# brian-kelley/CUDA-QR

Hardware: AMD Instinct MI355X
Metric: fp64 GFLOP/s (% of roofline) + ||A-QR||_F/||A||_F, m x n QR at 1/2/4/8 GPUs (higher is better)
Workload: dtype f64; 1 GPU; C3: 16384x16384 square fp64 QR on 1 MI355X, nb=256; m=16384, n=16384, m_per_gpu=16384, nb=256, ib=32, input_buffers=31, input=uniform[0,1) counter-hash generator, seed 12+i, resident in HBM, collective=none

## Files before the change

### cuda-qr_amd/__init__.py

```python
import ctypes as C
import os

import numpy as np

HERE = os.path.dirname(os.path.abspath(__file__))
_which = os.environ.get("CUDA_QR_AMD_LIB", "")
LAB = _which == "lab" or _which.endswith(".so")
LAB_LIB_PATH = os.path.join(HERE, "libmi355xqr_lab.so")
LIB_PATH = (os.path.join(HERE, _which) if _which.endswith(".so") else LAB_LIB_PATH) if LAB else os.path.join(HERE, "libmi355xqr.so")
HEADER = os.path.join(os.path.dirname(HERE), "include", "mi355x_qr.h")

if not os.path.exists(LIB_PATH):
    raise ImportError(
        f"{LIB_PATH} is missing: build it with `make -C {HERE} all lab` (or python -c 'import __graft_entry__ as g; "
        "g.build()').  The HIP extension is mandatory; there is no CPU fallback.")

try:
    import torch
except Exception:
    pass

lib = C.CDLL(LIB_PATH)

QR_PROF_CLASSES = 4
# ... 243 lines not shown
_sig("qr_plan_get_profile", C.c_int, _vp, C.POINTER(Profile))
_sig("qr_plan_get_profile_records", C.c_int, _vp, C.c_int, C.POINTER(C.c_int), _dp, _dp)
_sig("qr_device_info", C.c_int, C.c_char_p, C.c_int, C.POINTER(C.c_int), C.POINTER(C.c_int), C.POINTER(C.c_size_t))
_sig("qr_probe_mfma_f64_tflops", C.c_int, _dp)
_sig("qr_probe_copy_gbps", C.c_int, _dp)
_sig("qrd_gemm_nn", C.c_int, _vp, C.c_int, C.c_int, C.c_int, C.c_double, _vp, C.c_int, _vp, C.c_int, C.c_double,
     _vp, C.c_int)
_sig("qrd_gemm_tn", C.c_int, _vp, C.c_int, C.c_int, C.c_int, C.c_double, _vp, C.c_int, _vp, C.c_int, C.c_double,
     _vp, C.c_int, _vp, C.c_size_t, _vp, C.c_int)
_sig("qrd_gemm_tn_update", C.c_int, _vp, C.c_int, C.c_int, C.c_int, C.c_double, _vp, C.c_int, _vp, C.c_int, C.c_double,
     _vp, C.c_int, _vp, C.c_size_t)
_sig("qrd_gemm_tn_update_wide", C.c_int, _vp, C.c_int, C.c_int, C.c_int, C.c_double, _vp, C.c_int, _vp, C.c_int, C.c_double,
     _vp, C.c_int, _vp, C.c_size_t)
if hasattr(lib, "qrd_gemm_tn_update_even"):
    _sig("qrd_gemm_tn_update_even", C.c_int, _vp, C.c_int, C.c_int, C.c_int, C.c_double, _vp, C.c_int, _vp, C.c_int, C.c_double,
         _vp, C.c_int, _vp, C.c_size_t, C.c_int)
    _sig("qrd_tn_even_launches", C.c_longlong)
    _sig("qrd_tn_even_last_grid", C.c_int)
if hasattr(lib, "qrd_gemm_nn_tri"):
    _sig("qrd_gemm_nn_tri", C.c_int, _vp, C.c_int, C.c_int, C.c_int, C.c_double, _vp, C.c_int, _vp, C.c_int, C.c_double,
         _vp, C.c_int)
    _sig("qrd_gemm_nn_tri_tile", C.c_int, _vp, C.c_int, C.c_int, C.c_int, C.c_int, _vp, C.c_int, _vp, C.c_int, _vp, C.c_int)
    _sig("qrd_vt_tri_launches", C.c_longlong)
_sig("qrd_gemm_tn_dual", C.c_int, _vp, C.c_int, C.c_int, C.c_int, _vp, C.c_int, _vp, C.c_int, _vp, C.c_int, _vp, C.c_int, _vp, C.c_int, _vp, C.c_int,
     _vp, C.c_size_t)
_sig("qrd_trsm_gt", C.c_int, _vp, C.c_int, C.c_int, _vp, C.c_int, _vp, C.c_int, _vp, C.c_int, _vp, C.c_int)
_sig("qrd_larft", C.c_int, _vp, C.c_int, C.c_int, _vp, C.c_int, _vp, _vp, C.c_int, _vp, C.c_int, _vp, C.c_int)
_sig("qrd_panel_ws_size", C.c_size_t, C.c_int)
_sig("qrd_panel_tsqr", C.c_int, _vp, _vp, C.c_int, C.c_int, C.c_int, _vp, _vp, C.c_int, _vp, C.c_int, _vp, C.c_int)
_sig("qrd_panel_cholqr", C.c_int, _vp, _vp, C.c_int, C.c_int, C.c_int, _vp, _vp, C.c_int, _vp, C.c_int, _vp, C.c_int, _vp, _vp, C.c_size_t, C.c_int)
_sig("qrd_leaf_update_gram", C.c_int, _vp, C.c_int, C.c_int, _vp, C.c_int, _vp, _vp, C.c_int, _vp, C.c_size_t, C.c_int, C.POINTER(C.c_int))
_sig("qrd_gemm_nt", C.c_int, _vp, C.c_int, C.c_int, C.c_int, C.c_int, _vp, C.c_int, _vp, C.c_int, _vp, C.c_int, C.c_int, _vp)
if hasattr(lib, "qrd_gemm_nt4_ok"):
    _sig("qrd_gemm_nt4_ok", C.c_int, C.c_int, C.c_int, C.c_int, _vp, C.c_int, _vp, C.c_int, _vp, C.c_int)
_sig("qrd_transpose", C.c_int, _vp, C.c_int, C.c_int, _vp, C.c_int, _vp, C.c_int)
_sig("qrd_copy_block", C.c_int, _vp, _vp, C.c_int, _vp, C.c_int, C.c_int, C.c_int)
_sig("qrd_init", C.c_int)
_sig("qrd_device_sync", C.c_int)


def strerror(rc):
    return lib.qr_strerror(rc).decode()


def check(rc, what=""):
    if rc != 0:
# ... 1484 lines not shown
```

### cuda-qr_amd/csrc/qr_host.c

```c
#define _POSIX_C_SOURCE 200809L
#include <pthread.h>
#include <sched.h>
#include <stdint.h>
#include <stdio.h>
#include <stdlib.h>
#include <string.h>
#include <time.h>

#include "../../include/mi355x_qr.h"
#include "qr_device.h"
#include "qr_plan_internal.h"

#define CHECK(x) do { int rc_ = (x); if (rc_) return rc_; } while (0)

#define QR_MAX_NB 512
#define QR_HALF 256
#define QR_DEFAULT_SPLIT "64"
#define QR_DEFAULT_SPLIT_BIG "32"

#define QR_MAX_DEVICES 64
static pthread_mutex_t g_lock = PTHREAD_MUTEX_INITIALIZER;
static int g_nb = 0, g_ib = 0;
static int g_nb_explicit = 0;
static unsigned char g_dev_inited[QR_MAX_DEVICES];

#define QR_FUSE_NN_MIN_ROWS 20000
#define QR_TFOLD_MAX 128
#define QR_EARLY_W1 4096
#define QR_TAIL_TC_MS 0.0

typedef struct qr_knobs {
    int fuse_nn;
    int split_t;
    int early_next;
    int plan_cache;
    int early_product;
    int fused_panel;
    int fused_min_rows;
    int tsqr_halves_rows;
    int cqr_min_rows;
    int tall_nt;
    int cqr_park;
    int cqr_min_rows_la;
    int cqr_retry;
    int trsm_next;
    int defer_t;
    int fused_gram;
} qr_knobs;
static qr_knobs g_knobs;
static pthread_once_t g_knobs_once = PTHREAD_ONCE_INIT;
// ... 249 lines not shown
        const char* b = lab_getenv("MI355XQR_BALANCE");
        p->bal_rp = 14.0; p->bal_ru = 44.0; p->bal_tc0 = 1.1; p->bal_tc1 = 0.6;
        if (p->npairs) {
            int cus = 256;
            qrd_device_info(NULL, 0, &cus, NULL, NULL);
            const int pc = qrd_stream_cus(p->s_pair[0][0]);
            p->bal_rp = 0.22 * pc; p->bal_ru = 0.244 * (cus - pc);
        }
        if (b) {
            p->bal_rp = 0.0;
            sscanf(b, "%lf,%lf,%lf,%lf", &p->bal_rp, &p->bal_ru, &p->bal_tc0, &p->bal_tc1);
        }
        {
            const char* tt = lab_getenv("MI355XQR_TAILTC");
            p->bal_tail_tc = tt ? atof(tt) : QR_TAIL_TC_MS;
        }
        p->bal_auto = (b == NULL) && p->npairs > 1;
        p->bal_tc0_base = p->bal_tc0; p->bal_tc1_base = p->bal_tc1;
    }
    for (int e = 0; e < 2 && !rc; ++e) rc = qrd_event_create_notiming(&p->ev_v[e]);
    for (int e = 0; e < 2 && !rc; ++e) {
        rc = qrd_event_create_notiming(&p->ev_panel[e]);
        if (!rc) rc = qrd_event_create_notiming(&p->ev_wide[e]);
        if (!rc) rc = qrd_event_create_notiming(&p->ev_tree[e]);
    }
    size_t cap = (size_t) 256 * nb * (size_t) n;
    if (cap > ((size_t) 16 << 20)) cap = (size_t) 16 << 20;
    if (cap < ((size_t) 1 << 16)) cap = (size_t) 1 << 16;
    p->slab_cap = cap;
    p->w_cap = (size_t) nb * n;
    for (int e = 0; e < 2 && !rc; ++e) {
        rc = qrd_malloc((void**) &p->Vw2[e], sizeof(double) * (size_t) p->ldv * nb);
        if (!rc) rc = qrd_malloc((void**) &p->VT2[e], sizeof(double) * (size_t) p->ldv * nb);
        if (!rc) rc = qrd_malloc((void**) &p->T2[e], sizeof(double) * (size_t) nb * nb);
        if (!rc) rc = qrd_memset(p->stream, p->T2[e], 0, sizeof(double) * (size_t) nb * nb);
        if (!rc) rc = qrd_memset(p->stream, p->Vw2[e], 0, sizeof(double) * (size_t) p->ldv * nb);
    }
    p->Vw = p->Vw2[0]; p->VT = p->VT2[0]; p->T = p->T2[0];
    if (!rc) rc = qrd_malloc((void**) &p->W, sizeof(double) * p->w_cap);
    if (!rc) rc = qrd_malloc((void**) &p->Wn, sizeof(double) * (size_t) nb * nb);
    if (!rc && p->npairs && p->bal_rp > 0.0) rc = qrd_malloc((void**) &p->We, sizeof(double) * p->w_cap);
    if (!rc && p->We) rc = qrd_malloc((void**) &p->Ye, sizeof(double) * p->w_cap);
    if (!rc) rc = qrd_malloc((void**) &p->Yn, sizeof(double) * (size_t) nb * nb);
    if (!rc && (size_t) n * 8 <= (size_t) m) rc = qrd_malloc((void**) &p->Ye2, sizeof(double) * p->w_cap);
    if (!rc) rc = qrd_malloc((void**) &p->slabs_u, sizeof(double) * p->slab_cap);
    if (!rc) rc = qrd_malloc((void**) &p->Tt, sizeof(double) * (size_t) nb * nb);
    if (!rc) rc = qrd_malloc((void**) &p->G, sizeof(double) * (size_t) nb * nb);
    if (!rc) rc = qrd_malloc((void**) &p->X, sizeof(double) * (size_t) nb * nb);
    if (!rc) rc = qrd_malloc((void**) &p->slabs, sizeof(double) * p->slab_cap);
    {
        const char* pa = getenv("MI355XQR_PANEL");
        p->panel_tsqr = (pa && strcmp(pa, "tsqr") == 0) ? 1 : 3;
    }
    if (!rc) rc = qrd_malloc((void**) &p->panel_ws, sizeof(double) * qrd_panel_ws_size(m));
    if (!rc && p->panel_tsqr == 3) rc = qrd_malloc((void**) &p->chol_ws, sizeof(double) * QRD_CHOLQR_WS);
    if (!rc && p->panel_tsqr == 3 && knobs()->early_product) {
        p->slab_ep_cap = (size_t) 32 * (size_t) (nb > 64 ? nb : 64) * 128;
        rc = qrd_malloc((void**) &p->slabs_ep, sizeof(double) * p->slab_ep_cap);
    }
    if (!rc && p->panel_tsqr == 3 && knobs()->fused_panel) {
        if (knobs()->cqr_min_rows > 0 && m >= plan_cqr_min_rows(p)) {
            rc = qrd_malloc((void**) &p->cq_ws, sizeof(double) * qrd_panel_cqr_ws_doubles());
            if (!rc) rc = qrd_malloc((void**) &p->cq_status, 4 * sizeof(int));
            if (!rc) rc = qrd_memset(p->stream, p->cq_status, 0, 4 * sizeof(int));
            if (!rc) rc = qrd_host_word_alloc(&p->cq_hword, &p->cq_hword_dev);
            {
                const char* gm = getenv("MI355XQR_GUARD");
                p->guard_latch = gm != NULL && strcmp(gm, "latch") == 0;
            }
        }
        if (!rc) rc = qrd_malloc((void**) &p->pf_ws, sizeof(double) * qrd_panel_fused_ws_doubles());
        if (!rc) rc = qrd_memset(p->stream, p->pf_ws, 0, sizeof(double) * qrd_panel_fused_ws_doubles());
        if (!rc) rc = qrd_malloc((void**) &p->pf_status, 4 * sizeof(int));
        if (!rc) rc = qrd_memset(p->stream, p->pf_status, 0, 4 * sizeof(int));
    }
    if (!rc && (p->m != p->m_user || p->n != p->n_user)) rc = qrd_malloc((void**) &p->padA, sizeof(double) * (size_t) p->m * p->n);
    if (!rc && p->n != p->n_user) rc = qrd_malloc((void**) &p->pad_tau, sizeof(double) * (size_t) p->n);
    if (rc) { qr_plan_destroy(p); return rc; }
    *out = p;
    return 0;
}

int qr_plan_destroy(qr_plan* p)
{
    if (!p) return 0;
    qr_plan_sync(p);
    qrd_graph_destroy(p->graph_exec);
    for (int e = 0; e < 2; ++e) {
        if (p->ev_panel[e]) qrd_event_destroy(p->ev_panel[e]);
        if (p->ev_v[e]) qrd_event_destroy(p->ev_v[e]);
        if (p->ev_wide[e]) qrd_event_destroy(p->ev_wide[e]);
        if (p->ev_tree[e]) qrd_event_destroy(p->ev_tree[e]);
        qrd_free(p->Vw2[e]); qrd_free(p->VT2[e]); qrd_free(p->T2[e]);
    }
    qrd_free(p->Wn); qrd_free(p->slabs_u); qrd_free(p->We); qrd_free(p->Ye); qrd_free(p->Yn); qrd_free(p->Ye2);
    for (int i = 0; i < p->npairs; ++i)
        for (int j = 0; j < 2; ++j)
            if (p->s_pair[i][j] && !(j == 1 && p->pair_shared_u[i])) qrd_stream_destroy(p->s_pair[i][j]);
    if (p->npairs == 0 && p->stream_u) qrd_stream_destroy(p->stream_u);
    for (int e = 0; e < 2; ++e) {
        if (p->ev_hop[e]) qrd_event_destroy(p->ev_hop[e]);
        if (p->ev_extra[e]) qrd_event_destroy(p->ev_extra[e]);
        if (p->ev_next[e]) qrd_event_destroy(p->ev_next[e]);
        if (p->ev_half[e]) qrd_event_destroy(p->ev_half[e]);
    }
    for (int i = 0; i < 2 * p->prof_cap; ++i)
        if (p->prof_ev && p->prof_ev[i]) qrd_event_destroy(p->prof_ev[i]);
    free(p->prof_ev); free(p->prof_cls); free(p->prof_flops); free(p->prof_bytes);
    qrd_free(p->W); qrd_free(p->Tt); qrd_free(p->G); qrd_free(p->X);
    qrd_free(p->slabs); qrd_free(p->panel_ws); qrd_free(p->chol_ws); qrd_free(p->slabs_ep);
    qrd_free(p->pf_ws); qrd_free(p->pf_status); qrd_free(p->cq_ws); qrd_free(p->cq_status); qrd_free(p->padA); qrd_free(p->pad_tau);
    qrd_host_word_free(p->cq_hword);
    qrd_free(p->pv_d); qrd_free(p->pv_i); qrd_free(p->pv_scatter);
    qrd_free(p->sv_d); qrd_free(p->sv_i); qrd_free(p->sv_t); free(p->sv_h);
    qrd_free(p->hd_status);
    if (p->s_main) qrd_stream_destroy(p->s_main);
    free(p);
    return 0;
}

static int plan_read_status(qr_plan* p)
{
    int rc = 0;
    if (p->pf_dirty && p->pf_status) {
        int st[4] = {0, 0, 0, 0};
        CHECK(qrd_d2h(p->s_main, st, p->pf_status, sizeof st));
        CHECK(qrd_stream_sync(p->s_main));
        p->pf_dirty = 0;
        if (st[0] || st[1]) {
            CHECK(qrd_memset(p->s_main, p->pf_status, 0, sizeof st));
            CHECK(qrd_stream_sync(p->s_main));
        }
// ... 334 lines not shown
        if (!need_t) continue;
        if (p->v_ready && nhalf == 1) CHECK(qrd_event_record(p->v_ready, p->stream));
        double* Vh = p->Vw + (size_t) c0 * ldv + c0;
        double* Thh = p->T + (size_t) c0 * ldt + c0;
        if (wh > ib && !cqr_done && p->defer_hint && fused_half && nhalf == 1 && !gram_done) {
            p->t_deferred = 1;
            continue;
        }
        if (wh > ib && !cqr_done) {
            double* Ghh = p->G + (size_t) c0 * nb + c0;
            if (!gram_done) CHECK(tn(p, wh, wh, mk - c0, Vh, ldv, Vh, ldv, Ghh, nb, NULL));
            if (!t_merged) CHECK(qrd_larft(p->stream, wh, ib, Ghh, nb, dtau + k + c0, Thh, ldt, NULL, 0, p->X, nb));
        }
        if (h > 0) {
            double* G12 = p->G + (size_t) c0 * nb;
            CHECK(tn(p, c0, wh, mk - c0, p->Vw + c0, ldv, Vh, ldv, G12, nb, NULL));
            CHECK(qrd_gemm_nn(p->stream, c0, wh, wh, 1.0, G12, nb, Thh, ldt, 0.0, p->X, c0));
            CHECK(qrd_gemm_nn(p->stream, c0, wh, c0, -1.0, p->T, ldt, p->X, c0, 0.0, p->T + (size_t) c0 * ldt, ldt));
        }
    }
    return 0;
}

static void use_set(qr_plan* p, int e) { p->Vw = p->Vw2[e]; p->VT = p->VT2[e]; p->T = p->T2[e]; }

static int apply_small_t(qr_plan* p, void* stream, const double* V, int ldv, const double* T, int ldt, int mk, int kw, double* A2,
                         int lda, int nc, double* Wbuf, double* Ybuf, double* slabs)
{
    void* const t_wait = p->t_wait;
    p->t_wait = NULL;
    const int fold_max = QR_TFOLD_MAX;
    if (kw <= fold_max && slabs != NULL) {
        if (t_wait) CHECK(qrd_stream_wait_event(stream, t_wait));
        CHECK(qrd_gemm_tn(stream, kw, nc, mk, 1.0, V, ldv, A2, lda, 0.0, Wbuf, kw, slabs, p->slab_cap, T, ldt));
    } else {
        CHECK(qrd_gemm_tn(stream, kw, nc, mk, 1.0, V, ldv, A2, lda, 0.0, Ybuf, kw, slabs, p->slab_cap, NULL, 0));
        if (t_wait) CHECK(qrd_stream_wait_event(stream, t_wait));
        CHECK(qrd_gemm_tn(stream, kw, nc, kw, 1.0, T, ldt, Ybuf, kw, 0.0, Wbuf, kw, NULL, 0, NULL, 0));
    }
    return apply_vw(p, stream, V, ldv, mk, kw, A2, lda, nc, Wbuf, Ybuf);
}

static int apply_vw(qr_plan* p, void* stream, const double* V, int ldv, int mk, int kw, double* A2, int lda, int nc, double* Wbuf, double* Ybuf)
{
    (void) p;
    if (knobs()->tall_nt && Ybuf && mk >= 16384 && kw >= 32 && kw % 16 == 0 && nc >= 128) {
        const int r = nc % 64, ni = nc - r;
// ... 108 lines not shown
    if (!p->npairs || p->bal_rp <= 0.0 || nwide <= 0) return 0;
    const double F = 4.0 * mk * (double) wout * 1e-9;
    const double tc = chain_ms(p, mk, wout);
    const double x = (F * nwide / p->bal_ru - tc) / (F * (1.0 / p->bal_rp + 1.0 / p->bal_ru));
    int xi = (int) x;
    xi -= xi % 128;
    if (xi < 128) return 0;
    return xi > nwide ? nwide : xi;
}

static int update_bound(const qr_plan* p, int mk, int wout, int nwide)
{
    if (!p->npairs || p->bal_ru <= 0.0 || nwide <= 0) return 0;
    const double F = 4.0 * mk * (double) wout * 1e-9;
    const double tc = chain_ms(p, mk, wout);
    return F * nwide / p->bal_ru > tc;
}

static int deferred_gram(qr_plan* p, void* stream, int e, int mk, int wout, double* slabs)
{
#ifdef QR_TRACE_DEFER
    fprintf(stderr, "deferred_t_merge: mk %d wout %d on %s\n", mk, wout, stream == p->stream_u ? "update stream" : "panel stream");
#endif
    return qrd_gemm_tn(stream, wout, wout, mk, 1.0, p->Vw2[e], p->ldv, p->Vw2[e], p->ldv, 0.0, p->G, p->nb, slabs, p->slab_cap, NULL, 0);
}
static int deferred_tree(qr_plan* p, void* stream, int e, int wout, const double* tau_k)
{
    return qrd_larft(stream, wout, p->ib, p->G, p->nb, tau_k, p->T2[e], p->ldt, NULL, 0, p->X, p->nb);
}
static int deferred_t_merge(qr_plan* p, void* stream, int e, int mk, int wout, const double* tau_k, double* slabs)
{
    CHECK(deferred_gram(p, stream, e, mk, wout, slabs));
    return deferred_tree(p, stream, e, wout, tau_k);
}

static int lookahead_update_no_t(qr_plan* p, void* stream, int e, double* dA, int lda, int k, int mk, int wout, int nc, double* slabs)
{
    double* A2 = dA + (size_t) (k + wout) * lda + k;
    if (wout % 32 || wout > 256 || nc % 16 || nc < 16 || p->ib != 32) return 1;
    CHECK(prof_begin_on(p, 4, stream));
    CHECK(qrd_gemm_tn(stream, wout, nc, mk, 1.0, p->Vw2[e], p->ldv, A2, lda, 0.0, p->Yn, wout, slabs, p->slab_cap, NULL, 0));
    CHECK(qrd_trsm_gt(stream, wout, nc, p->G, p->nb, p->T2[e], p->ldt, p->Yn, wout, p->Wn, wout));
    CHECK(apply_vw(p, stream, p->Vw2[e], p->ldv, mk, wout, A2, lda, nc, p->Wn, p->Yn));
    CHECK(prof_end(p, 4.0 * mk * (double) nc * wout, 24.0 * mk * (double) nc + 16.0 * mk * wout));
    return 0;
}

static int geqrf_issue(qr_plan* p, double* dA, int m, int n, int lda, double* dtau);

int qr_geqrf_dev(qr_plan* p, double* dA, int m, int n, int lda, double* dtau)
{
    if (!p || !dA || !dtau || n < 1 || m < n || m > p->m || n > p->n || lda < m) return QR_E_ARG;
    if (!p->padA && m == p->m_user && n == p->n_user && m >= 512 && !p->use_graph && !p->pad_failed && ((lda & 1) || ((uintptr_t) dA & 15)) &&
        (double) p->m * p->n * 8.0 <= 4294967296.0) {
        if (qrd_malloc((void**) &p->padA, sizeof(double) * (size_t) p->m * p->n)) { p->padA = NULL; p->pad_failed = 1; }
    }
    if (p->padA && m == p->m_user && n == p->n_user && !p->use_graph) {
        const int mp = p->m, np = p->n;
        CHECK(qrd_memset(p->stream, p->padA, 0, sizeof(double) * (size_t) mp * np));
        CHECK(qrd_copy_block(p->stream, dA, lda, p->padA, mp, m, n));
        if (np > n) CHECK(qrd_set_identity(p->stream, p->padA + (size_t) n * mp + m, mp, np - n, np - n, 0));
        CHECK(geqrf_issue(p, p->padA, mp, np, mp, np > n ? p->pad_tau : dtau));
        if (np > n) CHECK(qrd_d2d(p->stream, dtau, p->pad_tau, sizeof(double) * (size_t) n));
        return qrd_copy_block(p->stream, p->padA, mp, dA, lda, m, n);
    }
// ... 26 lines not shown
    void* ns = i < 0 ? p->s_main : p->s_pair[i][0];
    void* nu = i < 0 ? NULL : p->s_pair[i][1];
    CHECK(qrd_event_record(p->ev_hop[0], p->stream));
    CHECK(qrd_stream_wait_event(ns, p->ev_hop[0]));
    if (p->stream_u && p->stream_u != nu) {
        CHECK(qrd_event_record(p->ev_hop[1], p->stream_u));
        CHECK(qrd_stream_wait_event(nu ? nu : ns, p->ev_hop[1]));
    }
    p->stream = ns; p->stream_u = nu; p->pair_cur = i;
    if (i >= 0 && p->bal_auto) {
        int cus = 256;
        qrd_device_info(NULL, 0, &cus, NULL, NULL);
        const int pc = qrd_stream_cus(ns);
        const int uc = nu ? qrd_stream_cus(nu) : cus;
        p->bal_rp = 0.22 * (pc < cus ? pc : 32);
        p->bal_ru = 0.244 * uc;
        const double f = pc <= 32 ? 1.0 : (pc <= 64 ? 0.8 : 0.7);
        p->bal_tc0 = p->bal_tc0_base * f; p->bal_tc1 = p->bal_tc1_base * f;
    }
    return 0;
}

static int geqrf_issue_inner(qr_plan* p, double* dA, int m, int n, int lda, double* dtau);

static int geqrf_issue(qr_plan* p, double* dA, int m, int n, int lda, double* dtau)
{
    const int rc = geqrf_issue_inner(p, dA, m, n, lda, dtau);
    if (rc) {
        p->stream = p->s_main;
        p->stream_u = p->npairs ? NULL : p->stream_u;
        p->pair_cur = -1;
        use_set(p, 0);
    }
    return rc;
}

static int geqrf_issue_inner(qr_plan* p, double* dA, int m, int n, int lda, double* dtau)
{
    const int nb = p->nb;
    p->cq_parked = 0;
    p->park_hint = 0;
    p->defer_hint = 0;
    p->t_deferred = 0;
    if (!p->lookahead) {
        use_set(p, 0);
        for (int k = 0, wout = 0; k < n; k += wout) {
            wout = imin(nb, n - k);
            if (p->ib == 32 && wout > 32 && wout % 32 != 0) wout -= wout % 32;
            const int mk = m - k, nt = n - (k + wout);
            CHECK(prof_begin(p, 2));
            p->park_hint = nt == 0 || ((size_t) nt * 8 <= (size_t) mk && p->Ye2 != NULL);
            CHECK(factor_panel(p, dA, m, lda, k, wout, dtau, nt > 0, NULL));
            CHECK(prof_end(p, 2.0 * mk * (double) wout * wout, 16.0 * mk * wout));
            if (nt > 0) CHECK(update_cols(p, p->stream, 0, dA, lda, k, mk, wout, k + wout, nt, p->W, NULL, p->slabs, 1, 1));
            CHECK(cq_unpark(p));
        }
        return 0;
    }
    int wide_pending[2] = {0, 0}, extra_pending = 0;
    int v_recorded[2] = {0, 0};
    int t_deferred[2] = {0, 0};
    const int split_t = knobs()->split_t;
    const int early_env = knobs()->early_next, early_w1 = QR_EARLY_W1;
    int early_done = 0;
    {
        const int w0 = imin(nb, n);
        use_set(p, 0);
        CHECK(prof_begin(p, 2));
        p->v_ready = (split_t && p->npairs > 0 && w0 <= QR_HALF && n > w0) ? p->ev_v[0] : NULL;
        v_recorded[0] = p->v_ready != NULL;
        CHECK(factor_panel(p, dA, m, lda, 0, w0, dtau, n > w0, NULL));
        p->v_ready = NULL;
        CHECK(prof_end(p, 2.0 * m * (double) w0 * w0, 16.0 * m * w0));
        CHECK(qrd_event_record(p->ev_panel[0], p->stream));
    }
    CHECK(enter_phase(p, phase_of(p, n, n)));
    int s = 0;
    for (int k = 0; k < n; k += nb, ++s) {
        const int e = s & 1, wout = imin(nb, n - k), mk = m - k, nt = n - (k + wout);
        if (nt <= 0) break;
        const int wnext = imin(nb, nt), nwide = nt - wnext;
// ... 4 lines not shown
        CHECK(enter_phase(p, phase_now));
        int extra = p->We ? balance_cols(p, mk, wout, nwide) : 0;
        const int k1 = k + wout, mk1 = m - k1, nt1 = n - (k1 + wnext);
        const int wnext2 = nt1 > 0 ? imin(nb, nt1) : 0;
        const int early_next = early_env && p->npairs > 0 && p->stream_u != NULL && nhalf2 == 0 && wnext2 > 0 && wnext2 <= QR_HALF &&
                               nwide > wnext2 && update_bound(p, mk, wout, nwide) &&
                               update_bound(p, mk1, wnext, nt1 - wnext2) && phase_of(p, nt1, n) == phase_now;
        if (early_next && extra > nwide - wnext2) { extra = nwide - wnext2; extra -= extra % 128; }
        const int n_on_u = !n_early && p->stream_u != NULL && p->npairs > 0 &&
                           (p->next_on_update == 1 || (p->next_on_update == 2 && !update_bound(p, mk, wout, nwide)));
        if (t_deferred[e] && !n_on_u) {
            CHECK(deferred_t_merge(p, p->stream, e, mk, wout, dtau + k, p->slabs));
            CHECK(qrd_event_record(p->ev_panel[e], p->stream));
            t_deferred[e] = 0;
        }
        if (n_early) {
        } else if (n_on_u && t_deferred[e]) {
            CHECK(qrd_stream_wait_event(p->stream_u, v_recorded[e] ? p->ev_v[e] : p->ev_panel[e]));
            if (extra_pending) CHECK(qrd_stream_wait_event(p->stream_u, p->ev_extra[e ^ 1]));
            CHECK(prof_begin_on(p, 3, p->stream_u));
            CHECK(deferred_gram(p, p->stream_u, e, mk, wout, p->slabs_u));
            CHECK(prof_end(p, 2.0 * mk * (double) wout * wout, 8.0 * mk * wout));
            t_deferred[e] = 0;
            int need_tree_first = !knobs()->trsm_next;
            if (!need_tree_first) {
                const int rc = lookahead_update_no_t(p, p->stream_u, e, dA, lda, k, mk, wout, nfirst, p->slabs_u);
                if (rc < 0 || rc > 1) return rc;
                need_tree_first = rc == 1;
            }
            if (need_tree_first) {
                CHECK(deferred_tree(p, p->stream_u, e, wout, dtau + k));
                CHECK(update_cols(p, p->stream_u, e, dA, lda, k, mk, wout, k + wout, nfirst, p->Wn, p->Yn, p->slabs_u, 0, 0));
            }
            CHECK(qrd_event_record(p->ev_next[e], p->stream_u));
            CHECK(qrd_stream_wait_event(p->stream, p->ev_next[e]));
            if (!need_tree_first) {
                CHECK(deferred_tree(p, p->stream_u, e, wout, dtau + k));
                CHECK(qrd_event_record(p->ev_tree[e], p->stream_u));
                CHECK(qrd_stream_wait_event(p->stream, p->ev_tree[e]));
            }
            wide_pending[e ^ 1] = 0;
        } else if (n_on_u) {
            if (v_recorded[e]) {
                CHECK(qrd_stream_wait_event(p->stream_u, p->ev_v[e]));
                p->t_wait = p->ev_panel[e];
            } else
                CHECK(qrd_stream_wait_event(p->stream_u, p->ev_panel[e]));
            if (extra_pending) CHECK(qrd_stream_wait_event(p->stream_u, p->ev_extra[e ^ 1]));
            CHECK(update_cols(p, p->stream_u, e, dA, lda, k, mk, wout, k + wout, nfirst, p->Wn, p->Yn, p->slabs_u, 0, 0));
            p->t_wait = NULL;
            CHECK(qrd_event_record(p->ev_next[e], p->stream_u));
            CHECK(qrd_stream_wait_event(p->stream, p->ev_next[e]));
            wide_pending[e ^ 1] = 0;
        } else {
            if (s > 0 && wide_pending[e ^ 1]) {
                CHECK(qrd_stream_wait_event(p->stream, p->ev_wide[e ^ 1]));
                wide_pending[e ^ 1] = 0;
            }
            CHECK(update_cols(p, p->stream, e, dA, lda, k, mk, wout, k + wout, nfirst, p->Wn, p->Yn, p->slabs, 0, 0));
        }
        const int wide_cols = nhalf2 + nwide - extra;
        const int cw = k + wout + wnext;
        if (wide_cols > 0) {
// ... 39 lines not shown
        CHECK(prof_begin(p, 2));
        p->v_ready = (split_t && p->npairs > 0 && wnext <= QR_HALF && nt1 > 0) ? p->ev_v[e ^ 1] : NULL;
        v_recorded[e ^ 1] = p->v_ready != NULL;
        {
            const int nwide1 = nt1 - wnext2;
            const double w_ms = 4.0 * mk * (double) wout * (double) wide_cols * 1e-9 / (p->bal_ru > 0.0 ? p->bal_ru : 50.0);
            const int n_on_u1 = !early_next && p->stream_u != NULL && p->npairs > 0 &&
                                (p->next_on_update == 1 || (p->next_on_update == 2 && !update_bound(p, mk1, wnext, nwide1)));
            p->defer_hint = knobs()->defer_t && n_on_u1 && nt1 > 0 && wnext <= QR_HALF && w_ms < 0.75 * 0.45 * (double) wnext / 256.0 &&
                            phase_of(p, nt1, n) == phase_now;
        }
        CHECK(factor_panel(p, dA, m, lda, k1, wnext, dtau, nt1 > 0, nhalf2 > 0 ? p->ev_half[e] : NULL));
        p->defer_hint = 0;
        t_deferred[e ^ 1] = p->t_deferred;
        p->t_deferred = 0;
        p->v_ready = NULL;
        CHECK(prof_end(p, 2.0 * mk1 * (double) wnext * wnext, 16.0 * mk1 * wnext));
        CHECK(qrd_event_record(p->ev_panel[e ^ 1], p->stream));
        if (early_next) {
            CHECK(qrd_stream_wait_event(p->stream, p->ev_half[e]));
            CHECK(update_cols(p, p->stream, e ^ 1, dA, lda, k1, mk1, wnext, k1 + wnext, imin(QR_HALF, wnext2), p->Wn, p->Yn, p->slabs, 0, 0));
            early_done = 1;
        }
        if (extra > 0) {
            CHECK(update_cols(p, p->stream, e, dA, lda, k, mk, wout, early_next ? cw + nwide - extra : cw, extra, p->We, p->Ye,
                              p->slabs, 2, 0));
            CHECK(qrd_event_record(p->ev_extra[e], p->stream));
            extra_pending = 1;
        }
    }
    for (int e = 0; e < 2; ++e)
        if (wide_pending[e]) CHECK(qrd_stream_wait_event(p->stream, p->ev_wide[e]));
    use_set(p, 0);
    return enter_phase(p, -1);
}

int qr_applyq_dev(qr_plan* p, const double* dA, int m, int n, int lda, const double* dtau, double* dC, int ccols,
                  int ldc, int identity_start)
{
    if (!p || !dA || !dtau || !dC || n < 1 || m < n || m > p->m || n > p->n || ccols < 1 || ldc < m) return QR_E_ARG;
    const int nb = p->nb, ib = p->ib, ldv = p->ldv, ldt = p->ldt;
    CHECK(ensure_w(p, (size_t) nb * ccols));
    use_set(p, 0);
    if (identity_start) CHECK(qrd_set_identity(p->stream, dC, ldc, m, ccols, 0));
    const int npan = (n + nb - 1) / nb;
    for (int pi = npan - 1; pi >= 0; --pi) {
        const int k = pi * nb, wout = imin(nb, n - k), mk = m - k;
        const int c0 = identity_start ? k : 0, nc = ccols - c0;
        if (nc <= 0) continue;
        const double* Ak = dA + (size_t) k * lda + k;
        CHECK(qrd_extract_v(p->stream, Ak, lda, mk, wout, p->Vw, ldv));
        CHECK(tn(p, wout, wout, mk, p->Vw, ldv, p->Vw, ldv, p->G, nb, NULL));
        CHECK(qrd_larft(p->stream, wout, ib, p->G, nb, dtau + k, p->T, ldt, p->Tt, 1, p->X, nb));
        CHECK(qrd_gemm_nn(p->stream, mk, wout, wout, 1.0, p->Vw, ldv, p->Tt, ldt, 0.0, p->VT, ldv));
        double* Cs = dC + (size_t) c0 * ldc + k;
        CHECK(tn(p, wout, nc, mk, p->VT, ldv, Cs, ldc, p->W, wout, NULL));
        CHECK(qrd_gemm_nn(p->stream, mk, nc, wout, -1.0, p->Vw, ldv, p->W, wout, 1.0, Cs, ldc));
// ... 822 lines not shown
}

int qr_tsqr_is_pipelined(qr_tsqr_plan* t) { return t && t->pipe_ok && t->nranks > 1; }

int qr_tsqr_set_schedule(qr_tsqr_plan* t, int mode)
{
    if (!t || mode < 0 || mode > 2) return QR_E_ARG;
    if (t->nranks < 2) return 0;
    CHECK(qr_tsqr_sync(t));
    if (mode == 1 && !t->pipe_able) return QR_E_ARG;
    if (mode == 2) { t->pipe_ok = t->pipe_able && t->pipe_env_on; t->pipe_auto = t->pipe_env_auto; t->pipe_calls = 0; t->pipe_fell_back = 0; }
    else { t->pipe_ok = mode; t->pipe_auto = 0; }
    t->stats_valid = 0;
    return 0;
}

int qr_tsqr_factor_dev(qr_tsqr_plan* t, double* dA, int lda, double* dR)
{
    if (!t || !dA || !dR || lda < t->m_local) return QR_E_ARG;
    if (t->nranks > 1 && !t->comm) return QR_E_ARG;
    if (t->nranks > 1 && t->pipe_ok && t->pipe_auto && t->pipe_calls == QR_TSQR_DECIDE_CALL) CHECK(tsqr_decide(t, 0));
    if (t->nranks > 1 && t->pipe_ok) return tsqr_factor_pipelined(t, dA, lda, dR, 0);
    if (t->nranks == 1) {
        CHECK(qr_geqrf_dev(t->p, dA, t->m_local, t->n, lda, t->dtau));
        CHECK(qr_extract_r_dev(t->p, dA, t->m_local, t->n, lda, dR, t->n, t->n));
        t->local_done = 0;
        return 0;
    }
    CHECK(qr_tsqr_local_dev(t, dA, lda));
    CHECK(qrd_allgather_f64(t->comm, t->p->s_main, t->dRp, t->dRall, (size_t) t->n * t->n));
    return qr_tsqr_stacked_dev(t, dR);
}

int qr_tsqr_formq_dev(qr_tsqr_plan* t, const double* dA, int lda, double* dQ, int ldq)
{
    if (!t || !dA || !dQ || lda < t->m_local || ldq < t->m_local) return QR_E_ARG;
    const int n = t->n, rows = t->m_local, sm = t->sm;
    qr_plan* p = t->p;
    if (t->nranks == 1) return qr_applyq_dev(p, dA, rows, n, lda, t->dtau, dQ, n, ldq, 1);
    qr_plan* p2 = t->p2;
    if (t->ev_q && t->q_pending) { CHECK(qrd_stream_wait_event(p2->s_main, t->ev_q)); t->q_pending = 0; }
    CHECK(qr_applyq_dev(p2, t->dS, sm, n, sm, t->dtau2, t->dQt, n, sm, 1));
    CHECK(qrd_event_record(t->ev_stacked, p2->s_main));
    CHECK(qrd_stream_wait_event(p->s_main, t->ev_stacked));
    t->stacked_pending = 0;
    CHECK(qrd_zero_block(p->s_main, dQ, ldq, rows, n));
    CHECK(qrd_copy_block(p->s_main, t->dQt + (size_t) t->rank * n, sm, dQ, ldq, n, n));
    CHECK(qrd_event_record(t->ev_q, p->s_main));
// ... 106 lines not shown
```

### cuda-qr_amd/csrc/qr_kernels.hip

```cpp
#include <hip/hip_runtime.h>
#include <stdint.h>
#include <string.h>
#include <stdlib.h>
#include <utility>
#include <mutex>
#include "qr_device.h"
#include "qr_common.h"
#include "qr_gemm_tile.h"
#include "qr_tn_even.h"
#include <atomic>

#define HIPCHK(x) do { hipError_t e_ = (x); if (e_ != hipSuccess) return (int) e_; } while (0)

template <int TI, int TJ, bool FAST>
__device__ __forceinline__ void gemm_nn_body(int M, int N, int K, double alpha, const double* __restrict__ A, int lda,
                                             const double* __restrict__ B, int ldb, double beta,
                                             double* __restrict__ C, int ldc, int jb, int kend)
{
    constexpr int BM = 32 * TI, BN = 32 * TJ, LA = BM + 16;
    extern __shared__ __attribute__((aligned(16))) double smem[];
    double* As = smem;
    double* Bs = smem + 2 * BK * LA;
    const int tid = threadIdx.x, lane = tid & 63, wave = tid >> 6;
    const int wi = wave & 1, wj = wave >> 1;
// ... 434 lines not shown
        for (int c = c0; c < c1; ++c) {
            double* r = R + (size_t) c * ldr + i;
            if (pair) *reinterpret_cast<v2d*>(r) = (v2d){0.0, 0.0}; else *r = 0.0;
        }
        return;
    }
#pragma unroll
    for (int q = 0; q < XR_COLS; ++q) {
        const int c = c0 + q;
        if (c >= c1) break;
        const double* a = A + (size_t) c * lda + i;
        v2d v = (v2d){0.0, 0.0};
        if (i + 1 <= c && i + 1 < m) v = *reinterpret_cast<const v2d*>(a);
        else if (i <= c && i < m) v[0] = a[0];
        double* r = R + (size_t) c * ldr + i;
        if (pair) *reinterpret_cast<v2d*>(r) = v; else *r = v[0];
    }
}

__global__ void extract_r_block_kernel(const double* __restrict__ A, int lda, int k, int w, double* __restrict__ R, int ldr, int rrows)
{
    const int i = blockIdx.x * blockDim.x + threadIdx.x, j = blockIdx.y;
    if (i < rrows && j < w) R[(size_t) j * ldr + i] = (i <= k + j) ? A[(size_t) (k + j) * lda + i] : 0.0;
}

__global__ void set_identity_kernel(double* __restrict__ C, int ld, int rows, int cols, int row_off)
{
    const int i = blockIdx.x * blockDim.x + threadIdx.x, c = blockIdx.y;
    if (i < rows && c < cols) C[(size_t) c * ld + i] = (i + row_off == c) ? 1.0 : 0.0;
}

__global__ void copy_block_kernel(const double* __restrict__ S, int lds, double* __restrict__ D, int ldd, int rows, int cols)
{
    const int i = blockIdx.x * blockDim.x + threadIdx.x, c = blockIdx.y;
    if (i < rows && c < cols) D[(size_t) c * ldd + i] = S[(size_t) c * lds + i];
}

__global__ void copy_blocks_kernel(const double* __restrict__ S, int lds, size_t sstride, double* __restrict__ D, int ldd, size_t dstride, int rows, int cols)
{
    const int i = blockIdx.x * blockDim.x + threadIdx.x, c = blockIdx.y;
    const size_t q = blockIdx.z;
    if (i < rows && c < cols) D[q * dstride + (size_t) c * ldd + i] = S[q * sstride + (size_t) c * lds + i];
}

__host__ __device__ __forceinline__ double hash_uniform(uint64_t seed, uint64_t idx)
{
// ... 758 lines not shown

int qrd_extract_v(void* stream, const double* P, int ld, int mk, int w, double* V, int ldv)
{
    hipLaunchKernelGGL(extract_v_kernel, dim3((mk + 255) / 256, w), dim3(256), 0, (hipStream_t) stream, P, ld, mk, w,
                       V, ldv);
    return (int) hipGetLastError();
}

int qrd_extract_r(void* stream, const double* A, int lda, int m, int n, double* R, int ldr, int rrows)
{
    if (vec_ok(A, lda) && vec_ok(R, ldr)) {
        hipLaunchKernelGGL(extract_r_v2_kernel, dim3((rrows + 511) / 512, (n + XR_COLS - 1) / XR_COLS), dim3(256), 0, (hipStream_t) stream, A,
                           lda, m, n, R, ldr, rrows);
        return (int) hipGetLastError();
    }
    hipLaunchKernelGGL(extract_r_kernel, dim3((rrows + 255) / 256, n), dim3(256), 0, (hipStream_t) stream, A, lda, m,
                       n, R, ldr, rrows);
    return (int) hipGetLastError();
}

int qrd_extract_r_block(void* stream, const double* A, int lda, int k, int w, double* R, int ldr, int rrows)
{
    if (w <= 0 || rrows <= 0) return 0;
    hipLaunchKernelGGL(extract_r_block_kernel, dim3((rrows + 255) / 256, w), dim3(256), 0, (hipStream_t) stream, A, lda, k, w, R, ldr, rrows);
    return (int) hipGetLastError();
}

int qrd_set_identity(void* stream, double* C, int ld, int rows, int cols, int row_off)
{
    if (rows <= 0 || cols <= 0) return 0;
    hipLaunchKernelGGL(set_identity_kernel, dim3((rows + 255) / 256, cols), dim3(256), 0, (hipStream_t) stream, C, ld,
                       rows, cols, row_off);
    return (int) hipGetLastError();
}

int qrd_copy_block(void* stream, const double* S, int lds, double* D, int ldd, int rows, int cols)
{
    if (rows <= 0 || cols <= 0) return 0;
    hipLaunchKernelGGL(copy_block_kernel, dim3((rows + 255) / 256, cols), dim3(256), 0, (hipStream_t) stream, S, lds,
                       D, ldd, rows, cols);
    return (int) hipGetLastError();
}

int qrd_copy_blocks(void* stream, const double* S, int lds, size_t sstride, double* D, int ldd, size_t dstride, int rows, int cols, int batch)
{
    if (rows <= 0 || cols <= 0 || batch <= 0) return 0;
// ... 265 lines not shown
```

### cuda-qr_amd/csrc/qr_plan_internal.h

```cpp
#ifndef QR_PLAN_INTERNAL_H
#define QR_PLAN_INTERNAL_H
#include <stddef.h>
#include "../../include/mi355x_qr.h"

#define QR_MAX_PAIRS 4
struct qr_plan {
    int m, n, nb, ib, ldv, ldt;
    int use_graph;
    void* graph_exec;
    double *g_dA, *g_dtau; int g_m, g_n, g_lda;
    int lookahead;
    void* stream;
    void* stream_u;
    void* s_main;
    int npairs, pair_cur;
    void* s_pair[QR_MAX_PAIRS][2];
    int pair_shared_u[QR_MAX_PAIRS];
    double pair_until[QR_MAX_PAIRS];
    void* ev_hop[2];
    void* ev_extra[2];
    double *We, *Ye;
    double *Ye2;
    int m_user, n_user;
    double* pad_tau;
    int pad_failed;
    double* padA;
    double *Yn;
    double bal_rp, bal_ru, bal_tc0, bal_tc1;
    double bal_tail_tc;
    double bal_tc0_base, bal_tc1_base; int bal_auto;
    void* ev_half[2];
    void* ev_next[2];
    int next_on_update;
    void* ev_panel[2];
    void* t_wait;
    void* ev_v[2];
    void* v_ready;
    int defer_hint, t_deferred;
    void* ev_wide[2];
    void* ev_tree[2];
    double *Vw, *VT, *T;
    double *Vw2[2], *VT2[2], *T2[2];
    int vt_formed[2];
    double *W, *Wn, *Tt, *G, *X, *slabs, *slabs_u, *panel_ws;
    double* slabs_ep;
    size_t slab_ep_cap;
    int panel_tsqr;
    double* chol_ws;
    double* cq_ws; int* cq_status;
    int park_hint, cq_parked, cq_park_lda, cq_park_w;
    double* cq_park_top;
    unsigned *cq_hword, *cq_hword_dev;
    unsigned cq_seq;
    int guard_latch;
    int cq_dirty, pf_dirty;
    int fused_off;
    long long n_cqr, n_cqr_refused, n_pf_leaf_fallback, n_pf_stall;
    long long n_cqr_retried, n_cqr_retry_ok;
    double* pf_ws;
    unsigned pf_epoch;
    int* pf_status;
    size_t slab_cap, w_cap;
    int prof_on, prof_mask, prof_count, prof_cap, prof_open, prof_paused;
    void** prof_ev;
    void* prof_stream;
    int* prof_cls;
    double *prof_flops, *prof_bytes;
    double* pv_d;
    int* pv_i;
    double* pv_scatter;
    size_t pv_scatter_cap;
    double* sv_d;
    int* sv_i;
    int* sv_h;
    double* sv_t;
    size_t sv_t_cap;
    int* hd_status;
};

struct qr_lsacc {
    qr_plan* p;
    int n, nrhs;
    long long rows;
    double *buf, *R, *Rc, *Z, *T, *tau, *ssq;
    double* dd_buf;
};

struct qr_lsacc_batched {
    qr_plan* p;
    int n, nrhs, batch;
    double *R, *Z, *rss;
    int* rows;
};

typedef struct host_slot {
    int used, busy, cached, dev, m, n, nb;
    unsigned long long stamp;
    qr_plan* p;
    double *dA, *dtau, *dQ, *dR;
    size_t q_cap, r_cap;
} host_slot;

// ... 7 lines not shown
```

Baseline: 52160 GFLOP/s.

## Sink R extraction per panel into idle stream slots during factorization

Instead of extracting R after the full geqrf, R column blocks are copied into the output buffer incrementally during the factorization. Each step picks either the update stream or the panel stream based on a simple cost model, and the leftover blocks are flushed at the end. G and X are now double-buffered per lookahead set so that the deferred tree no longer needs the ev_tree event sync, and a vectorized 2-wide extract_r kernel is added. This adds scheduling heuristics with hardcoded timing constants, and the copies may contend with the critical path.

```diff
diff --git a/cuda-qr_amd/__init__.py b/cuda-qr_amd/__init__.py
--- a/cuda-qr_amd/__init__.py
+++ b/cuda-qr_amd/__init__.py
@@ -289,6 +289,8 @@
          _vp, C.c_int)
     _sig("qrd_gemm_nn_tri_tile", C.c_int, _vp, C.c_int, C.c_int, C.c_int, C.c_int, _vp, C.c_int, _vp, C.c_int, _vp, C.c_int)
     _sig("qrd_vt_tri_launches", C.c_longlong)
+if hasattr(lib, "qr_r_by_panel_launches"):
+    _sig("qr_r_by_panel_launches", C.c_longlong)
 _sig("qrd_gemm_tn_dual", C.c_int, _vp, C.c_int, C.c_int, C.c_int, _vp, C.c_int, _vp, C.c_int, _vp, C.c_int, _vp, C.c_int, _vp, C.c_int, _vp, C.c_int,
      _vp, C.c_size_t)
 _sig("qrd_trsm_gt", C.c_int, _vp, C.c_int, C.c_int, _vp, C.c_int, _vp, C.c_int, _vp, C.c_int, _vp, C.c_int)
diff --git a/cuda-qr_amd/csrc/qr_host.c b/cuda-qr_amd/csrc/qr_host.c
--- a/cuda-qr_amd/csrc/qr_host.c
+++ b/cuda-qr_amd/csrc/qr_host.c
@@ -26,6 +26,7 @@
 
 #define QR_FUSE_NN_MIN_ROWS 20000
 #define QR_TFOLD_MAX 128
+#define QR_RSINK_PER_STEP 3
 #define QR_EARLY_W1 4096
 #define QR_TAIL_TC_MS 0.0
 
@@ -321,7 +322,6 @@
     for (int e = 0; e < 2 && !rc; ++e) {
         rc = qrd_event_create_notiming(&p->ev_panel[e]);
         if (!rc) rc = qrd_event_create_notiming(&p->ev_wide[e]);
-        if (!rc) rc = qrd_event_create_notiming(&p->ev_tree[e]);
     }
     size_t cap = (size_t) 256 * nb * (size_t) n;
     if (cap > ((size_t) 16 << 20)) cap = (size_t) 16 << 20;
@@ -344,8 +344,9 @@
     if (!rc && (size_t) n * 8 <= (size_t) m) rc = qrd_malloc((void**) &p->Ye2, sizeof(double) * p->w_cap);
     if (!rc) rc = qrd_malloc((void**) &p->slabs_u, sizeof(double) * p->slab_cap);
     if (!rc) rc = qrd_malloc((void**) &p->Tt, sizeof(double) * (size_t) nb * nb);
-    if (!rc) rc = qrd_malloc((void**) &p->G, sizeof(double) * (size_t) nb * nb);
-    if (!rc) rc = qrd_malloc((void**) &p->X, sizeof(double) * (size_t) nb * nb);
+    if (!rc) rc = qrd_malloc((void**) &p->G2[0], sizeof(double) * (size_t) nb * nb);
+    if (!rc) rc = qrd_malloc((void**) &p->X2[0], sizeof(double) * (size_t) nb * nb);
+    p->G = p->G2[0]; p->X = p->X2[0];
     if (!rc) rc = qrd_malloc((void**) &p->slabs, sizeof(double) * p->slab_cap);
     {
         const char* pa = getenv("MI355XQR_PANEL");
@@ -375,6 +376,8 @@
     }
     if (!rc && (p->m != p->m_user || p->n != p->n_user)) rc = qrd_malloc((void**) &p->padA, sizeof(double) * (size_t) p->m * p->n);
     if (!rc && p->n != p->n_user) rc = qrd_malloc((void**) &p->pad_tau, sizeof(double) * (size_t) p->n);
+    if (!rc && p->lookahead) rc = qrd_malloc((void**) &p->G2[1], sizeof(double) * (size_t) nb * nb);
+    if (!rc && p->lookahead) rc = qrd_malloc((void**) &p->X2[1], sizeof(double) * (size_t) nb * nb);
     if (rc) { qr_plan_destroy(p); return rc; }
     *out = p;
     return 0;
@@ -389,8 +392,7 @@
         if (p->ev_panel[e]) qrd_event_destroy(p->ev_panel[e]);
         if (p->ev_v[e]) qrd_event_destroy(p->ev_v[e]);
         if (p->ev_wide[e]) qrd_event_destroy(p->ev_wide[e]);
-        if (p->ev_tree[e]) qrd_event_destroy(p->ev_tree[e]);
-        qrd_free(p->Vw2[e]); qrd_free(p->VT2[e]); qrd_free(p->T2[e]);
+        qrd_free(p->Vw2[e]); qrd_free(p->VT2[e]); qrd_free(p->T2[e]); qrd_free(p->G2[e]); qrd_free(p->X2[e]);
     }
     qrd_free(p->Wn); qrd_free(p->slabs_u); qrd_free(p->We); qrd_free(p->Ye); qrd_free(p->Yn); qrd_free(p->Ye2);
     for (int i = 0; i < p->npairs; ++i)
@@ -406,7 +408,7 @@
     for (int i = 0; i < 2 * p->prof_cap; ++i)
         if (p->prof_ev && p->prof_ev[i]) qrd_event_destroy(p->prof_ev[i]);
     free(p->prof_ev); free(p->prof_cls); free(p->prof_flops); free(p->prof_bytes);
-    qrd_free(p->W); qrd_free(p->Tt); qrd_free(p->G); qrd_free(p->X);
+    qrd_free(p->W); qrd_free(p->Tt);
     qrd_free(p->slabs); qrd_free(p->panel_ws); qrd_free(p->chol_ws); qrd_free(p->slabs_ep);
     qrd_free(p->pf_ws); qrd_free(p->pf_status); qrd_free(p->cq_ws); qrd_free(p->cq_status); qrd_free(p->padA); qrd_free(p->pad_tau);
     qrd_host_word_free(p->cq_hword);
@@ -787,7 +789,7 @@
     return 0;
 }
 
-static void use_set(qr_plan* p, int e) { p->Vw = p->Vw2[e]; p->VT = p->VT2[e]; p->T = p->T2[e]; }
+static void use_set(qr_plan* p, int e) { p->Vw = p->Vw2[e]; p->VT = p->VT2[e]; p->T = p->T2[e]; p->G = p->G2[e]; p->X = p->X2[e]; }
 
 static int apply_small_t(qr_plan* p, void* stream, const double* V, int ldv, const double* T, int ldt, int mk, int kw, double* A2,
                          int lda, int nc, double* Wbuf, double* Ybuf, double* slabs)
@@ -942,11 +944,11 @@
 #ifdef QR_TRACE_DEFER
     fprintf(stderr, "deferred_t_merge: mk %d wout %d on %s\n", mk, wout, stream == p->stream_u ? "update stream" : "panel stream");
 #endif
-    return qrd_gemm_tn(stream, wout, wout, mk, 1.0, p->Vw2[e], p->ldv, p->Vw2[e], p->ldv, 0.0, p->G, p->nb, slabs, p->slab_cap, NULL, 0);
+    return qrd_gemm_tn(stream, wout, wout, mk, 1.0, p->Vw2[e], p->ldv, p->Vw2[e], p->ldv, 0.0, p->G2[e], p->nb, slabs, p->slab_cap, NULL, 0);
 }
 static int deferred_tree(qr_plan* p, void* stream, int e, int wout, const double* tau_k)
 {
-    return qrd_larft(stream, wout, p->ib, p->G, p->nb, tau_k, p->T2[e], p->ldt, NULL, 0, p->X, p->nb);
+    return qrd_larft(stream, wout, p->ib, p->G2[e], p->nb, tau_k, p->T2[e], p->ldt, NULL, 0, p->X2[e], p->nb);
 }
 static int deferred_t_merge(qr_plan* p, void* stream, int e, int mk, int wout, const double* tau_k, double* slabs)
 {
@@ -960,7 +962,7 @@
     if (wout % 32 || wout > 256 || nc % 16 || nc < 16 || p->ib != 32) return 1;
     CHECK(prof_begin_on(p, 4, stream));
     CHECK(qrd_gemm_tn(stream, wout, nc, mk, 1.0, p->Vw2[e], p->ldv, A2, lda, 0.0, p->Yn, wout, slabs, p->slab_cap, NULL, 0));
-    CHECK(qrd_trsm_gt(stream, wout, nc, p->G, p->nb, p->T2[e], p->ldt, p->Yn, wout, p->Wn, wout));
+    CHECK(qrd_trsm_gt(stream, wout, nc, p->G2[e], p->nb, p->T2[e], p->ldt, p->Yn, wout, p->Wn, wout));
     CHECK(apply_vw(p, stream, p->Vw2[e], p->ldv, mk, wout, A2, lda, nc, p->Wn, p->Yn));
     CHECK(prof_end(p, 4.0 * mk * (double) nc * wout, 24.0 * mk * (double) nc + 16.0 * mk * wout));
     return 0;
@@ -1033,6 +1035,19 @@
 }
 
 static int geqrf_issue_inner(qr_plan* p, double* dA, int m, int n, int lda, double* dtau);
+
+static long long g_r_by_panel_launches;
+long long qr_r_by_panel_launches(void) { return __atomic_load_n(&g_r_by_panel_launches, __ATOMIC_RELAXED); }
+static int sink_r_pending(qr_plan* p, void* stream, const double* dA, int lda, int* r_next, int r_ready, int max_panels)
+{
+    for (int q = 0; q < max_panels && *r_next < r_ready; ++q) {
+        const int k = *r_next, w = imin(p->nb, r_ready - k);
+        CHECK(qrd_extract_r_block(stream, dA, lda, k, w, p->r_sink + (size_t) k * p->r_ldr, p->r_ldr, p->r_rrows));
+        __atomic_fetch_add(&g_r_by_panel_launches, 1, __ATOMIC_RELAXED);
+        *r_next = k + w;
+    }
+    return 0;
+}
 
 static int geqrf_issue(qr_plan* p, double* dA, int m, int n, int lda, double* dtau)
 {
@@ -1068,6 +1083,9 @@
         }
         return 0;
     }
+    const int r_by_panel = p->r_sink != NULL && dA != p->padA;
+    int r_next = 0;
+    if (r_by_panel) p->r_sunk = 1;
     int wide_pending[2] = {0, 0}, extra_pending = 0;
     int v_recorded[2] = {0, 0};
     int t_deferred[2] = {0, 0};
@@ -1118,7 +1136,7 @@
             CHECK(deferred_gram(p, p->stream_u, e, mk, wout, p->slabs_u));
             CHECK(prof_end(p, 2.0 * mk * (double) wout * wout, 8.0 * mk * wout));
             t_deferred[e] = 0;
-            int need_tree_first = !knobs()->trsm_next;
+            int need_tree_first = !knobs()->trsm_next || extra > 0;
             if (!need_tree_first) {
                 const int rc = lookahead_update_no_t(p, p->stream_u, e, dA, lda, k, mk, wout, nfirst, p->slabs_u);
                 if (rc < 0 || rc > 1) return rc;
@@ -1130,11 +1148,7 @@
             }
             CHECK(qrd_event_record(p->ev_next[e], p->stream_u));
             CHECK(qrd_stream_wait_event(p->stream, p->ev_next[e]));
-            if (!need_tree_first) {
-                CHECK(deferred_tree(p, p->stream_u, e, wout, dtau + k));
-                CHECK(qrd_event_record(p->ev_tree[e], p->stream_u));
-                CHECK(qrd_stream_wait_event(p->stream, p->ev_tree[e]));
-            }
+            if (!need_tree_first) CHECK(deferred_tree(p, p->stream_u, e, wout, dtau + k));
             wide_pending[e ^ 1] = 0;
         } else if (n_on_u) {
             if (v_recorded[e]) {
@@ -1220,6 +1234,18 @@
             CHECK(update_cols(p, p->stream, e ^ 1, dA, lda, k1, mk1, wnext, k1 + wnext, imin(QR_HALF, wnext2), p->Wn, p->Yn, p->slabs, 0, 0));
             early_done = 1;
         }
+        if (r_by_panel && extra == 0 && !early_next) {
+            const double w_ms = 4.0 * mk * (double) wout * (double) wide_cols * 1e-9 / (p->bal_ru > 0.0 ? p->bal_ru : 50.0);
+            const int one_launch = p->pf_ws && !p->fused_off && mk1 <= 8192 && mk1 >= knobs()->fused_min_rows;
+            const double p_ms = (one_launch ? 0.62 : 0.62 + 0.9 * (double) mk1 / 16384.0) * (double) wnext / 256.0;
+            if (w_ms < 0.75 * p_ms) {
+                if (p->stream_u && (n_on_u || wide_cols > 0)) CHECK(sink_r_pending(p, p->stream_u, dA, lda, &r_next, k1, QR_RSINK_PER_STEP));
+            } else {
+                const double x_ms = 16.0 * (double) p->r_rrows * (double) nb / 0.6e9;
+                const int fit = (int) ((w_ms - p_ms + 0.1) / x_ms);
+                CHECK(sink_r_pending(p, p->stream, dA, lda, &r_next, k1 + wnext, imin(fit, QR_RSINK_PER_STEP)));
+            }
+        }
         if (extra > 0) {
             CHECK(update_cols(p, p->stream, e, dA, lda, k, mk, wout, early_next ? cw + nwide - extra : cw, extra, p->We, p->Ye,
                               p->slabs, 2, 0));
@@ -1230,7 +1256,9 @@
     for (int e = 0; e < 2; ++e)
         if (wide_pending[e]) CHECK(qrd_stream_wait_event(p->stream, p->ev_wide[e]));
     use_set(p, 0);
-    return enter_phase(p, -1);
+    CHECK(enter_phase(p, -1));
+    if (r_by_panel) CHECK(sink_r_pending(p, p->stream, dA, lda, &r_next, n, n));
+    return 0;
 }
 
 int qr_applyq_dev(qr_plan* p, const double* dA, int m, int n, int lda, const double* dtau, double* dC, int ccols,
@@ -2099,8 +2127,13 @@
     if (t->nranks > 1 && t->pipe_ok && t->pipe_auto && t->pipe_calls == QR_TSQR_DECIDE_CALL) CHECK(tsqr_decide(t, 0));
     if (t->nranks > 1 && t->pipe_ok) return tsqr_factor_pipelined(t, dA, lda, dR, 0);
     if (t->nranks == 1) {
-        CHECK(qr_geqrf_dev(t->p, dA, t->m_local, t->n, lda, t->dtau));
-        CHECK(qr_extract_r_dev(t->p, dA, t->m_local, t->n, lda, dR, t->n, t->n));
+        qr_plan* const p = t->p;
+        p->r_sink = dR; p->r_ldr = t->n; p->r_rrows = t->n; p->r_sunk = 0;
+        const int rc = qr_geqrf_dev(p, dA, t->m_local, t->n, lda, t->dtau);
+        const int sunk = p->r_sunk;
+        p->r_sink = NULL; p->r_sunk = 0;
+        CHECK(rc);
+        if (!sunk) CHECK(qr_extract_r_dev(p, dA, t->m_local, t->n, lda, dR, t->n, t->n));
         t->local_done = 0;
         return 0;
     }
diff --git a/cuda-qr_amd/csrc/qr_kernels.hip b/cuda-qr_amd/csrc/qr_kernels.hip
--- a/cuda-qr_amd/csrc/qr_kernels.hip
+++ b/cuda-qr_amd/csrc/qr_kernels.hip
@@ -480,6 +480,31 @@
 {
     const int i = blockIdx.x * blockDim.x + threadIdx.x, j = blockIdx.y;
     if (i < rrows && j < w) R[(size_t) j * ldr + i] = (i <= k + j) ? A[(size_t) (k + j) * lda + i] : 0.0;
+}
+
+__global__ __launch_bounds__(256) void extract_r_block_v2_kernel(const double* __restrict__ A, int lda, int k, int w, double* __restrict__ R, int ldr, int rrows)
+{
+    const int i = 2 * (blockIdx.x * 256 + threadIdx.x), j0 = blockIdx.y * XR_COLS, j1 = min(w, j0 + XR_COLS);
+    if (i >= rrows) return;
+    const bool pair = i + 1 < rrows;
+    if ((int) blockIdx.x * 512 > k + j1 - 1) {
+        for (int j = j0; j < j1; ++j) {
+            double* r = R + (size_t) j * ldr + i;
+            if (pair) *reinterpret_cast<v2d*>(r) = (v2d){0.0, 0.0}; else *r = 0.0;
+        }
+        return;
+    }
+#pragma unroll
+    for (int q = 0; q < XR_COLS; ++q) {
+        const int j = j0 + q, c = k + j;
+        if (j >= j1) break;
+        const double* a = A + (size_t) c * lda + i;
+        v2d v = (v2d){0.0, 0.0};
+        if (i + 1 <= c) v = *reinterpret_cast<const v2d*>(a);
+        else if (i <= c) v[0] = a[0];
+        double* r = R + (size_t) j * ldr + i;
+        if (pair) *reinterpret_cast<v2d*>(r) = v; else *r = v[0];
+    }
 }
 
 __global__ void set_identity_kernel(double* __restrict__ C, int ld, int rows, int cols, int row_off)
@@ -1284,6 +1309,11 @@
 int qrd_extract_r_block(void* stream, const double* A, int lda, int k, int w, double* R, int ldr, int rrows)
 {
     if (w <= 0 || rrows <= 0) return 0;
+    if (vec_ok(A, lda) && vec_ok(R, ldr)) {
+        hipLaunchKernelGGL(extract_r_block_v2_kernel, dim3((rrows + 511) / 512, (w + XR_COLS - 1) / XR_COLS), dim3(256), 0, (hipStream_t) stream, A,
+                           lda, k, w, R, ldr, rrows);
+        return (int) hipGetLastError();
+    }
     hipLaunchKernelGGL(extract_r_block_kernel, dim3((rrows + 255) / 256, w), dim3(256), 0, (hipStream_t) stream, A, lda, k, w, R, ldr, rrows);
     return (int) hipGetLastError();
 }
diff --git a/cuda-qr_amd/csrc/qr_plan_internal.h b/cuda-qr_amd/csrc/qr_plan_internal.h
--- a/cuda-qr_amd/csrc/qr_plan_internal.h
+++ b/cuda-qr_amd/csrc/qr_plan_internal.h
@@ -38,11 +38,12 @@
     void* v_ready;
     int defer_hint, t_deferred;
     void* ev_wide[2];
-    void* ev_tree[2];
-    double *Vw, *VT, *T;
+    double *Vw, *VT, *T, *G, *X;
     double *Vw2[2], *VT2[2], *T2[2];
+    double *G2[2], *X2[2];
+    double* r_sink; int r_ldr, r_rrows, r_sunk;
     int vt_formed[2];
-    double *W, *Wn, *Tt, *G, *X, *slabs, *slabs_u, *panel_ws;
+    double *W, *Wn, *Tt, *slabs, *slabs_u, *panel_ws;
     double* slabs_ep;
     size_t slab_ep_cap;
     int panel_tsqr;
@@ -78,6 +79,8 @@
     int* hd_status;
 };
 
+long long qr_r_by_panel_launches(void);
+
 struct qr_lsacc {
     qr_plan* p;
     int n, nrhs;
```

Result: no change. 52640 GFLOP/s (median of 6 runs) (+0.9%).
